# tspooner/rl_markets

Hardware: AMD Instinct MI355X
Metric: env-steps/sec (whole node) at 65 536 parallel books (higher is better)
Workload: dtype f64

## Files before the change

rl_markets_amd/csrc/lob_env.h:

```cpp
#ifndef LOB_ENV_H
#define LOB_ENV_H

#include <hip/hip_runtime.h>

#include "lob_internal.h"
#include "lob_state.h"

LOB_HD int drec_pad4(int n) { return (n + 3) & ~3; }
LOB_HD int drec_words(int D, int T) { return 4 + 4 * drec_pad4(D) + drec_pad4(2 * T); }
LOB_HD int drec_ask_px(int, int) { return 4; }
LOB_HD int drec_ask_vol(int D, int) { return 4 + drec_pad4(D); }
LOB_HD int drec_bid_px(int D, int) { return 4 + 2 * drec_pad4(D); }
LOB_HD int drec_bid_vol(int D, int) { return 4 + 3 * drec_pad4(D); }
LOB_HD int drec_trades(int D, int) { return 4 + 4 * drec_pad4(D); }
LOB_HD void drec_from_abi(const uint32_t* src, int D, int T, uint32_t* dst) {
    const int Wd = drec_words(D, T);
    for (int i = 0; i < Wd; i++) dst[i] = 0;
    dst[0] = src[LOB_REC_TIME];
    dst[1] = src[LOB_REC_FLAGS];
    for (int l = 0; l < D; l++) {
        dst[drec_ask_px(D, T) + l] = src[lob_rec_ask_px(D, T) + l];
        dst[drec_ask_vol(D, T) + l] = src[lob_rec_ask_vol(D, T) + l];
        dst[drec_bid_px(D, T) + l] = src[lob_rec_bid_px(D, T) + l];
        dst[drec_bid_vol(D, T) + l] = src[lob_rec_bid_vol(D, T) + l];
// ... 70 lines not shown
    __device__ const uint32_t* row(int i) const { return rows + (size_t)i * (size_t)P.Wd; }
    __device__ const Track& track(int k) const { return S.track[(size_t)b * (size_t)S.track_len + (size_t)(k & S.track_mask)]; }
    __device__ const TrackHead& track_head(int k) const { return *reinterpret_cast<const TrackHead*>(&track(k)); }
    __device__ const TrackHead64& track_head64(int k) const { return *reinterpret_cast<const TrackHead64*>(&track(k)); }
    __device__ Track& track_w(int k) const { return S.track[(size_t)b * (size_t)S.track_len + (size_t)(k & S.track_mask)]; }
};

__device__ inline f64 key4(f64 p) { return rint(p * 10000.0); }

__device__ inline i64 cvt_long_x86(f64 d) {
    if (!(d >= -9223372036854775808.0 && d < 9223372036854775808.0)) return (i64)0x8000000000000000ull;
    return (i64)d;
}

struct OrderR {
    i64 size, qh, qt, ex;
};
__device__ inline i64 ord_remaining(const OrderR& o) { i64 r = o.size - o.ex; return r > 0 ? r : 0; }
__device__ inline bool ord_executed(const OrderR& o) { return o.ex >= o.size; }
__device__ inline i64 ord_transaction(OrderR& o, i64 volume) {
    i64 remaining_volume = volume - o.qh;
    if (remaining_volume > 0) {
        o.qh = 0;
        if (ord_remaining(o) <= remaining_volume) {
            o.ex = o.size;
            remaining_volume -= o.size;
        } else {
            o.ex += remaining_volume;
            remaining_volume = 0;
        }
    } else {
        o.qh -= volume;
    }
    return remaining_volume > 0 ? remaining_volume : 0;
}
__device__ inline void ord_cancellation(OrderR& o, i64 volume) {
    if (o.qt == 0) {
        o.qh -= volume;
    } else {
        f64 total = (f64)(o.qh + o.qt);
        i64 nh = cvt_long_x86((f64)o.qh - ceil((f64)(volume * o.qh) / total));
        i64 nt = cvt_long_x86((f64)o.qt - floor((f64)(volume * o.qt) / total));
        o.qh = nh;
        o.qt = nt;
    }
    if (o.qh < 0) {
        o.qt = (i64)((u64)o.qt + (u64)o.qh);
        o.qh = 0;
    }
    if (o.qt < 0) o.qt = 0;
}

__device__ inline void rm_push(const RMPtrs& r, int B, int b, f64 val) {
    i32 cnt = r.cnt[b], head = r.head[b];
    f64 sum = r.sum[b], mean = r.mean[b], s = r.s[b];
    sum += val;
    if (cnt < r.w) {
        head = (cnt == 0) ? 0 : (head + 1 == r.w ? 0 : head + 1);
        cnt++;
        r.ring[(size_t)head * B + b] = val;
        f64 n = (f64)cnt;
        f64 old_mean = mean;
        mean += (val - mean) / n;
        s += (val - mean) * (val - old_mean);
    } else {
        i32 oldest = head + 1 == r.w ? 0 : head + 1;
        f64 old = r.ring[(size_t)oldest * B + b];
        r.ring[(size_t)oldest * B + b] = val;
        head = oldest;
        f64 n = (f64)(cnt + 1);
        f64 old_mean = mean;
        mean += (val - mean) / n;
        s += (val - mean) * (val - old_mean);
        sum -= old;
        f64 n2 = (f64)cnt;
        f64 old_mean2 = mean;
        mean -= (old - mean) / n2;
        s -= (old - mean) * (old - old_mean2);
    }
    r.cnt[b] = cnt;
    r.head[b] = head;
    r.sum[b] = sum;
    r.mean[b] = mean;
    r.s[b] = s;
}
__device__ inline f64 rm_front(const RMPtrs& r, int B, int b) { return r.ring[(size_t)r.head[b] * B + b]; }
__device__ inline f64 rm_back(const RMPtrs& r, int B, int b) {
    i32 idx = r.head[b] - r.cnt[b] + 1;
    if (idx < 0) idx += r.w;
    return r.ring[(size_t)idx * B + b];
}
__device__ inline bool rm_full(const RMPtrs& r, int b) { return r.cnt[b] == r.w; }
__device__ inline f64 rm_std(const RMPtrs& r, int b) {
    f64 v = r.s[b] / (f64)(r.cnt[b] - 1);
    return v > 0 ? sqrt(v) : 0.0;
}
__device__ inline void acc_push(const AccPtrs& r, int B, int b, f64 val) {
    i32 cnt = r.cnt[b], head = r.head[b];
    f64 sum = r.sum[b];
    sum += val;
    if (cnt < r.w) {
        head = (cnt == 0) ? 0 : (head + 1 == r.w ? 0 : head + 1);
        cnt++;
        r.ring[(size_t)head * B + b] = val;
    } else {
        i32 oldest = head + 1 == r.w ? 0 : head + 1;
        f64 old = r.ring[(size_t)oldest * B + b];
        r.ring[(size_t)oldest * B + b] = val;
        head = oldest;
        sum -= old;
    }
    r.cnt[b] = cnt;
    r.head[b] = head;
    r.sum[b] = sum;
}

struct RMReg {
    i32 cnt, head, slot;
    f64 sum, mean, s, old;
};
__device__ inline void rm_load(const RMPtrs& r, int b, RMReg& g) {
    g.cnt = r.cnt[b]; g.head = r.head[b]; g.sum = r.sum[b]; g.mean = r.mean[b]; g.s = r.s[b];
}
__device__ inline void rm_prep(const RMPtrs& r, int B, int b, RMReg& g) {
    if (g.cnt < r.w) {
        g.slot = (g.cnt == 0) ? 0 : (g.head + 1 == r.w ? 0 : g.head + 1);
        g.old = 0.0;
    } else {
        g.slot = g.head + 1 == r.w ? 0 : g.head + 1;
        g.old = r.ring[(size_t)g.slot * B + b];
    }
}
__device__ inline void rm_apply(const RMPtrs& r, int B, int b, RMReg& g, f64 val) {
    g.sum += val;
    r.ring[(size_t)g.slot * B + b] = val;
    if (g.cnt < r.w) {
        g.cnt++;
        f64 n = (f64)g.cnt;
        f64 old_mean = g.mean;
        g.mean += (val - g.mean) / n;
        g.s += (val - g.mean) * (val - old_mean);
    } else {
        f64 n = (f64)(g.cnt + 1);
        f64 old_mean = g.mean;
        g.mean += (val - g.mean) / n;
        g.s += (val - g.mean) * (val - old_mean);
        g.sum -= g.old;
        f64 n2 = (f64)g.cnt;
        f64 old_mean2 = g.mean;
        g.mean -= (g.old - g.mean) / n2;
        g.s -= (g.old - g.mean) * (g.old - old_mean2);
    }
    g.head = g.slot;
    r.cnt[b] = g.cnt; r.head[b] = g.head; r.sum[b] = g.sum; r.mean[b] = g.mean; r.s[b] = g.s;
}
__device__ inline void rm_apply_reg(const RMPtrs& r, int B, int b, RMReg& g, f64 val) {
    g.sum += val;
    r.ring[(size_t)g.slot * B + b] = val;
    if (g.cnt < r.w) {
        g.cnt++;
        f64 n = (f64)g.cnt;
        f64 old_mean = g.mean;
        g.mean += (val - g.mean) / n;
        g.s += (val - g.mean) * (val - old_mean);
    } else {
        f64 n = (f64)(g.cnt + 1);
        f64 old_mean = g.mean;
        g.mean += (val - g.mean) / n;
        g.s += (val - g.mean) * (val - old_mean);
        g.sum -= g.old;
        f64 n2 = (f64)g.cnt;
        f64 old_mean2 = g.mean;
        g.mean -= (g.old - g.mean) / n2;
        g.s -= (g.old - g.mean) * (g.old - old_mean2);
    }
    g.head = g.slot;
}
__device__ inline void rm_store(const RMPtrs& r, int b, const RMReg& g) {
    r.cnt[b] = g.cnt; r.head[b] = g.head; r.sum[b] = g.sum; r.mean[b] = g.mean; r.s[b] = g.s;
}
struct AccReg {
    i32 cnt, head, slot;
    f64 sum, old;
};
__device__ inline void acc_load(const AccPtrs& r, int b, AccReg& g) { g.cnt = r.cnt[b]; g.head = r.head[b]; g.sum = r.sum[b]; }
__device__ inline void acc_prep(const AccPtrs& r, int B, int b, AccReg& g) {
    if (g.cnt < r.w) { g.slot = (g.cnt == 0) ? 0 : (g.head + 1 == r.w ? 0 : g.head + 1); g.old = 0.0; }
    else { g.slot = g.head + 1 == r.w ? 0 : g.head + 1; g.old = r.ring[(size_t)g.slot * B + b]; }
}
__device__ inline void acc_apply(const AccPtrs& r, int B, int b, AccReg& g, f64 val) {
    g.sum += val;
    r.ring[(size_t)g.slot * B + b] = val;
    if (g.cnt < r.w) g.cnt++;
    else g.sum -= g.old;
    g.head = g.slot;
    r.cnt[b] = g.cnt; r.head[b] = g.head; r.sum[b] = g.sum;
}

__device__ inline void acc_apply_reg(const AccPtrs& r, int B, int b, AccReg& g, f64 val) {
    g.sum += val;
    r.ring[(size_t)g.slot * B + b] = val;
    if (g.cnt < r.w) g.cnt++;
    else g.sum -= g.old;
    g.head = g.slot;
}
__device__ inline void acc_store(const AccPtrs& r, int b, const AccReg& g) { r.cnt[b] = g.cnt; r.head[b] = g.head; r.sum[b] = g.sum; }

__device__ inline f64 rec_price(const EnvCtx& c, int rec, int side, int l) {
    if (rec < 0) return 0.0;
    const uint32_t* r = c.row(rec);
    return (f64)__uint_as_float(r[(side == 0 ? drec_ask_px(c.P.D, c.P.T) : drec_bid_px(c.P.D, c.P.T)) + l]);
}
__device__ inline int book_level_of(const uint32_t* px, int D, f64 k) {
    uint32_t w[LOB_MAX_DEPTH];
    drec_levels(px, D, w);
    f32 p[LOB_MAX_DEPTH];
#pragma unroll
    for (int l = 0; l < LOB_MAX_DEPTH; l++) p[l] = l < D ? __uint_as_float(w[l]) : 0.0f;
    int hit = -1;
#pragma unroll
    for (int l = 0; l < LOB_MAX_DEPTH; l++)
        if (p[l] != 0.0f && key4((f64)p[l]) == k) hit = l;
    return hit;
}
__device__ inline i64 book_volume(const EnvCtx& c, int rec, int side, f64 price) {
    if (rec < 0) return 0;
    const uint32_t* r = c.row(rec);
    const uint32_t* px = r + (side == 0 ? drec_ask_px(c.P.D, c.P.T) : drec_bid_px(c.P.D, c.P.T));
    const uint32_t* vol = r + (side == 0 ? drec_ask_vol(c.P.D, c.P.T) : drec_bid_vol(c.P.D, c.P.T));
    const int hit = book_level_of(px, c.P.D, key4(price));
    return hit >= 0 ? (i64)(i32)vol[hit] : 0;
}
__device__ inline void book_volume2(const EnvCtx& c, int rec_a, int rec_b, int side, f64 price, i64& va, i64& vb) {
    const int opx = side == 0 ? drec_ask_px(c.P.D, c.P.T) : drec_bid_px(c.P.D, c.P.T);
    const int ovol = side == 0 ? drec_ask_vol(c.P.D, c.P.T) : drec_bid_vol(c.P.D, c.P.T);
    const uint32_t* ra = c.row(rec_a < 0 ? 0 : rec_a);
    const uint32_t* rb = c.row(rec_b < 0 ? 0 : rec_b);
    const int D = c.P.D;
    const f64 k = key4(price);
    uint32_t wa[LOB_MAX_DEPTH], wb[LOB_MAX_DEPTH];
    drec_levels(ra + opx, D, wa);
    drec_levels(rb + opx, D, wb);
    f32 pa[LOB_MAX_DEPTH], pb[LOB_MAX_DEPTH];
#pragma unroll
    for (int l = 0; l < LOB_MAX_DEPTH; l++) {
        pa[l] = l < D ? __uint_as_float(wa[l]) : 0.0f;
        pb[l] = l < D ? __uint_as_float(wb[l]) : 0.0f;
    }
    int ha = -1, hb = -1;
#pragma unroll
    for (int l = 0; l < LOB_MAX_DEPTH; l++) {
        if (pa[l] != 0.0f && key4((f64)pa[l]) == k) ha = l;
        if (pb[l] != 0.0f && key4((f64)pb[l]) == k) hb = l;
    }
    va = (rec_a >= 0 && ha >= 0) ? (i64)(i32)ra[ovol + ha] : 0;
    vb = (rec_b >= 0 && hb >= 0) ? (i64)(i32)rb[ovol + hb] : 0;
}

__device__ inline void order_volumes(const EnvCtx& c, const EnvR& e, int last_rec, int row_rec, i64& a_lv, i64& a_v,
                                     i64& b_lv, i64& b_v) {
    a_lv = a_v = b_lv = b_v = 0;
    const int D = c.P.D;
    const int apx = drec_ask_px(D, c.P.T), avol = drec_ask_vol(D, c.P.T);
    const int bpx = drec_bid_px(D, c.P.T), bvol = drec_bid_vol(D, c.P.T);
    const uint32_t* rl = c.row(last_rec < 0 ? 0 : last_rec);
    const uint32_t* rr = c.row(row_rec < 0 ? 0 : row_rec);
    const bool a_on = e.a_on != 0, b_on = e.b_on != 0;
    uint32_t wal[LOB_MAX_DEPTH], war[LOB_MAX_DEPTH], wbl[LOB_MAX_DEPTH], wbr[LOB_MAX_DEPTH];
    drec_levels(rl + apx, D, wal); drec_levels(rr + apx, D, war);
    drec_levels(rl + bpx, D, wbl); drec_levels(rr + bpx, D, wbr);
    f32 pal[LOB_MAX_DEPTH], par[LOB_MAX_DEPTH], pbl[LOB_MAX_DEPTH], pbr[LOB_MAX_DEPTH];
#pragma unroll
    for (int l = 0; l < LOB_MAX_DEPTH; l++) {
        pal[l] = (a_on && l < D) ? __uint_as_float(wal[l]) : 0.0f;
        par[l] = (a_on && l < D) ? __uint_as_float(war[l]) : 0.0f;
        pbl[l] = (b_on && l < D) ? __uint_as_float(wbl[l]) : 0.0f;
        pbr[l] = (b_on && l < D) ? __uint_as_float(wbr[l]) : 0.0f;
    }
    const f64 ka = key4(e.a_opx), kb = key4(e.b_opx);
    int hal = -1, har = -1, hbl = -1, hbr = -1;
#pragma unroll
    for (int l = 0; l < LOB_MAX_DEPTH; l++) {
        if (pal[l] != 0.0f && key4((f64)pal[l]) == ka) hal = l;
        if (par[l] != 0.0f && key4((f64)par[l]) == ka) har = l;
        if (pbl[l] != 0.0f && key4((f64)pbl[l]) == kb) hbl = l;
        if (pbr[l] != 0.0f && key4((f64)pbr[l]) == kb) hbr = l;
    }
    if (last_rec >= 0 && hal >= 0) a_lv = (i64)(i32)rl[avol + hal];
    if (row_rec >= 0 && har >= 0) a_v = (i64)(i32)rr[avol + har];
    if (last_rec >= 0 && hbl >= 0) b_lv = (i64)(i32)rl[bvol + hbl];
    if (row_rec >= 0 && hbr >= 0) b_v = (i64)(i32)rr[bvol + hbr];
}

struct RowFull {
    uint32_t apx[LOB_MAX_DEPTH], avol[LOB_MAX_DEPTH], bpx[LOB_MAX_DEPTH], bvol[LOB_MAX_DEPTH];
};
__device__ inline void row_full_load(const EnvCtx& c, int rec, RowFull& R) {
    const int D = c.P.D;
    const uint32_t* r = c.row(rec < 0 ? 0 : rec);
    drec_levels(r + drec_ask_px(D, c.P.T), D, R.apx);
    drec_levels(r + drec_ask_vol(D, c.P.T), D, R.avol);
    drec_levels(r + drec_bid_px(D, c.P.T), D, R.bpx);
    drec_levels(r + drec_bid_vol(D, c.P.T), D, R.bvol);
    const uint32_t keep = rec < 0 ? 0u : ~0u;
#pragma unroll
    for (int l = 0; l < LOB_MAX_DEPTH; l++) { R.apx[l] &= keep; R.avol[l] &= keep; R.bpx[l] &= keep; R.bvol[l] &= keep; }
}
__device__ inline void row_volumes(const EnvCtx& c, const EnvR& e, const RowFull& L, i64& a_v, i64& b_v) {
    const int D = c.P.D;
    const bool a_on = e.a_on != 0, b_on = e.b_on != 0;
    const f64 ka = key4(e.a_opx), kb = key4(e.b_opx);
    int ha = -1, hb = -1;
#pragma unroll
    for (int l = 0; l < LOB_MAX_DEPTH; l++) {
        const f32 pa = (a_on && l < D) ? __uint_as_float(L.apx[l]) : 0.0f;
        const f32 pb = (b_on && l < D) ? __uint_as_float(L.bpx[l]) : 0.0f;
        if (pa != 0.0f && key4((f64)pa) == ka) ha = l;
        if (pb != 0.0f && key4((f64)pb) == kb) hb = l;
    }
    uint32_t va = 0, vb = 0;
#pragma unroll
    for (int l = 0; l < LOB_MAX_DEPTH; l++) {
        if (l == ha) va = L.avol[l];
        if (l == hb) vb = L.bvol[l];
    }
    a_v = ha >= 0 ? (i64)(i32)va : 0;
    b_v = hb >= 0 ? (i64)(i32)vb : 0;
}

__device__ inline i64 full_volume(const EnvCtx& c, const RowFull& R, int side, f64 price) {
    const int D = c.P.D;
    const f64 k = key4(price);
    bool hit = false;
    uint32_t v = 0;
#pragma unroll
    for (int l = 0; l < LOB_MAX_DEPTH; l++) {
        const f32 p = l < D ? __uint_as_float(side == 0 ? R.apx[l] : R.bpx[l]) : 0.0f;
        if (p != 0.0f && key4((f64)p) == k) { hit = true; v = side == 0 ? R.avol[l] : R.bvol[l]; }
    }
    return hit ? (i64)(i32)v : 0;
}

__device__ inline void row_resolve(const EnvCtx&, const RowFull&) {}
__device__ inline f64 row_best_px(const RowFull& R, int side) { return (f64)__uint_as_float(side == 0 ? R.apx[0] : R.bpx[0]); }

#if defined(__HIP__)
struct RowLev {
    mutable uint4 q;
    mutable uint32_t apx, avol, bpx, bvol;
    uint32_t* stage;
    int li;
    mutable bool pending;
    bool none;
    __device__ __forceinline__ void resolve(const EnvCtx& c) const {
        if (!pending) return;
        const int D = c.P.D, D4 = drec_pad4(D);
        if (li < (c.P.Wd >> 2)) reinterpret_cast<uint4*>(stage)[li] = q;
        __builtin_amdgcn_fence(__ATOMIC_ACQ_REL, "workgroup", "local");
        __builtin_amdgcn_wave_barrier();
        const bool in = li < D && !none;
        const int l = li < D ? li : 0;
        const uint32_t a = stage[4 + l], av = stage[4 + D4 + l], b = stage[4 + 2 * D4 + l], bv = stage[4 + 3 * D4 + l];
        apx = in ? a : 0u; avol = in ? av : 0u; bpx = in ? b : 0u; bvol = in ? bv : 0u;
        __builtin_amdgcn_fence(__ATOMIC_ACQ_REL, "workgroup", "local");
        __builtin_amdgcn_wave_barrier();
        pending = false;
    }
};
__device__ __forceinline__ uint32_t grp_ballot(bool p) { return (uint32_t)(__ballot(p) >> (threadIdx.x & 48)) & 0xffffu; }
__device__ inline void row_full_load(const EnvCtx& c, int rec, RowLev& R) {
    const uint4* r = reinterpret_cast<const uint4*>(c.row(rec < 0 ? 0 : rec));
    const int nq = c.P.Wd >> 2;
    R.q = r[R.li < nq ? R.li : nq - 1];
    R.none = rec < 0;
    R.pending = true;
}
__device__ inline void row_resolve(const EnvCtx& c, const RowLev& R) { R.resolve(c); }
__device__ inline f64 row_best_px(const RowLev& R, int side) {
    return (f64)__uint_as_float(__shfl(side == 0 ? R.apx : R.bpx, 0, 16));
}
__device__ inline i64 rowlev_volume(const EnvCtx& c, const RowLev& R, int side, f64 k) {
    R.resolve(c);
    const f32 p = __uint_as_float(side == 0 ? R.apx : R.bpx);
    const uint32_t m = grp_ballot(p != 0.0f && key4((f64)p) == k);
    const uint32_t v = __shfl(side == 0 ? R.avol : R.bvol, m ? 31 - __clz(m) : 0, 16);
    return m ? (i64)(i32)v : 0;
}
__device__ inline i64 full_volume(const EnvCtx& c, const RowLev& R, int side, f64 price) { return rowlev_volume(c, R, side, key4(price)); }
__device__ inline void row_volumes_k(const EnvCtx& c, bool a_on, bool b_on, f64 ka, f64 kb, const RowLev& L, i64& a_v, i64& b_v) {
    const i64 va = rowlev_volume(c, L, 0, ka), vb = rowlev_volume(c, L, 1, kb);
    a_v = a_on ? va : 0;
    b_v = b_on ? vb : 0;
}
#endif

__device__ inline void check_orders(const DevParams& P, EnvR& e) {
    if (e.position >= P.pos_ub) e.b_on = 0;
    else if (e.position <= P.pos_lb) e.a_on = 0;
}

template <class ROW>
__device__ inline void place_one(const EnvCtx& c, EnvR& e, int side, f64 price, i32 price_ticks, const ROW& cur) {
    if (!(price > 0.0)) c.err(LOB_ERR_BAD_ORDER_PRICE);
    i64 qh = full_volume(c, cur, side, price);
    if (side == 0) {
        e.a_on = 1; e.a_opx = price; e.a_osz = c.P.order_size; e.a_oqh = qh; e.a_oqt = 0; e.a_oex = 0; e.a_oiq = qh; e.a_otk = price_ticks;
    } else {
        e.b_on = 1; e.b_opx = price; e.b_osz = c.P.order_size; e.b_oqh = qh; e.b_oqt = 0; e.b_oex = 0; e.b_oiq = qh; e.b_otk = price_ticks;
    }
}

template <class ROW>
__device__ inline void place_orders(const EnvCtx& c, EnvR& e, int al, int bl, const ROW& cur) {
    const DevParams& P = c.P;
    e.ask_level = al;
    e.bid_level = bl;
    int ta, tb;
    int band = 0, band_t = 0;
    if (P.quote_mode == LOB_QUOTE_BOOK) {
        row_resolve(c, cur);
        const f64 ap0 = row_best_px(cur, 0), bp0 = row_best_px(cur, 1);
        if (ap0 == 0.0 || bp0 == 0.0) c.err(LOB_ERR_UNDEF_PRICE);
        ta = lobh::to_ticks_hint((*c.tk), ap0, band) + al;
        tb = lobh::to_ticks_hint((*c.tk), bp0, band) - bl;
    } else {
        const Track& t = c.pre_prev ? *c.pre_prev : c.track(e.k - 1);
        f64 tp = t.tp_val;
        f64 half = t.spread_mean / 2.0;
        f64 half_spd = 0.0 > half ? 0.0 : half;
        ta = lobh::to_ticks_hint((*c.tk), tp + (f64)al * half_spd, band);
        tb = lobh::to_ticks_hint((*c.tk), tp - (f64)bl * half_spd, band);
    }
    e.ask_quote = lobh::to_price_hint((*c.tk), ta, band_t);
    e.bid_quote = lobh::to_price_hint((*c.tk), tb, band_t);
    place_one(c, e, 0, e.ask_quote, lobh::to_ticks_hint((*c.tk), e.ask_quote, band), cur);
    place_one(c, e, 1, e.bid_quote, lobh::to_ticks_hint((*c.tk), e.bid_quote, band), cur);
}
__device__ inline void place_orders(const EnvCtx& c, EnvR& e, int al, int bl) {
    RowFull cur;
    row_full_load(c, e.rec_cur, cur);
    place_orders(c, e, al, bl, cur);
}

__device__ inline void market_order(const EnvCtx& c, EnvR& e, i64 size, i64& out_vol, f64& out_proxy, f64& out_value, const RowFull& cur) {
    out_vol = 0; out_proxy = 0.0; out_value = 0.0;
    if (e.rec_cur < 0) c.err(LOB_ERR_UNDEF_PRICE);
    const f64 mip = e.mid;
    if (size == 0) return;
    const int side = size > 0 ? 0 : 1;
    i64 abs_size = size < 0 ? -size : size;
    i64 tv;
    if (e.done == 2) {
        tv = side == 0 ? c.S.prep[c.b].a_tv : c.S.prep[c.b].b_tv;
    } else {
        tv = c.pre_prev ? (side == 0 ? c.pre_prev->a_tv : c.pre_prev->b_tv) : (side == 0 ? c.track(e.k - 1).a_tv : c.track(e.k - 1).b_tv);
    }
    if (abs_size > tv) return;
    i64 executed = 0;
    f64 proxy = 0.0, value = 0.0;
    bool filled = false;
#pragma unroll
    for (int l = 0; l < LOB_MAX_DEPTH; l++) {
        const f32 pf = __uint_as_float(side == 0 ? cur.apx[l] : cur.bpx[l]);
        if (l >= c.P.D || filled || pf == 0.0f) continue;
        f64 p = (f64)pf;
        i64 lvol = (i64)(i32)(side == 0 ? cur.avol[l] : cur.bvol[l]);
        i64 left = abs_size - executed;
        i64 l_ex = lvol < left ? lvol : left;
        executed += l_ex;
        proxy -= (f64)l_ex * fabs(p - mip);
        if (side == 0) value -= (f64)l_ex * p;
        else value += (f64)l_ex * p;
        if (executed >= abs_size) {
            if (side == 0) e.a_ntr++; else e.b_ntr++;
            filled = true;
        }
    }
    out_vol = side == 0 ? executed : -executed;
    out_proxy = proxy;
    out_value = value;
}

#if defined(__HIP__)
__device__ inline void market_order(const EnvCtx& c, EnvR& e, i64 size, i64& out_vol, f64& out_proxy, f64& out_value, const RowLev& cur) {
    out_vol = 0; out_proxy = 0.0; out_value = 0.0;
    if (e.rec_cur < 0) c.err(LOB_ERR_UNDEF_PRICE);
    const f64 mip = e.mid;
    if (size == 0) return;
    const int side = size > 0 ? 0 : 1;
    const i64 abs_size = size < 0 ? -size : size;
    i64 tv;
    if (e.done == 2) tv = side == 0 ? c.S.prep[c.b].a_tv : c.S.prep[c.b].b_tv;
    else tv = c.pre_prev ? (side == 0 ? c.pre_prev->a_tv : c.pre_prev->b_tv) : (side == 0 ? c.track(e.k - 1).a_tv : c.track(e.k - 1).b_tv);
    if (abs_size > tv) return;
    cur.resolve(c);
    const f32 pf = __uint_as_float(side == 0 ? cur.apx : cur.bpx);
    const bool level = cur.li < c.P.D && pf != 0.0f;
    const i64 lvol = level ? (i64)(i32)(side == 0 ? cur.avol : cur.bvol) : 0;
    i64 incl = lvol;
#pragma unroll
    for (int d = 1; d < 16; d <<= 1) {
        const i64 up = __shfl_up(incl, d, 16);
        if (cur.li >= d) incl += up;
    }
    const i64 before = incl - lvol;
    const bool takes = level && before < abs_size;
    const i64 left = abs_size - before;
    const i64 l_ex = takes ? (lvol < left ? lvol : left) : 0;
    const uint32_t fills = grp_ballot(takes && before + l_ex >= abs_size);
    const i64 total = __shfl(incl, 15, 16);
    const i64 executed = total < abs_size ? total : abs_size;
    const f64 p = (f64)pf;
    const f64 t_proxy = takes ? (f64)l_ex * fabs(p - mip) : 0.0;
    const f64 t_value = takes ? (f64)l_ex * p : 0.0;
    f64 proxy = 0.0, value = 0.0;
    for (int l = 0; l < c.P.D; l++) {
        const f64 tp = __shfl(t_proxy, l, 16), tvl = __shfl(t_value, l, 16);
        proxy -= tp;
        if (side == 0) value -= tvl;
        else value += tvl;
    }
    if (fills) { if (side == 0) e.a_ntr++; else e.b_ntr++; }
    out_vol = side == 0 ? executed : -executed;
    out_proxy = proxy;
    out_value = value;
}
#endif

template <class ROW>
__device__ inline void clear_inventory(const EnvCtx& c, EnvR& e, const ROW& cur) {
    i64 v; f64 proxy, value;
    market_order(c, e, -e.position, v, proxy, value, cur);
    e.position += v;
    e.pnl_step += proxy;
    e.lo_vol_step += (i32)(v < 0 ? -v : v);
    e.ep_pnl += value;
    if (v > 0) e.market_buys++;
    else if (v < 0) e.market_sells++;
}
__device__ inline void clear_inventory(const EnvCtx& c, EnvR& e) {
    RowFull cur;
    row_full_load(c, e.rec_cur, cur);
    clear_inventory(c, e, cur);
}

template <class ROW>
__device__ inline void do_action(const EnvCtx& c, EnvR& e, int action, const ROW& cur) {
    int al, bl;
    switch (action) {
        case 0: al = 1; bl = 1; break;
        case 1: clear_inventory(c, e, cur); al = e.ask_level; bl = e.bid_level; break;
        case 2: al = 2; bl = 2; break;
        case 3: al = 3; bl = 3; break;
        case 4: al = 0; bl = 2; break;
        case 5: al = 2; bl = 0; break;
        case 6: al = 1; bl = 4; break;
        case 7: al = 4; bl = 1; break;
        case 8: al = 5; bl = 5; break;
        default: return;
    }
    place_orders(c, e, al, bl, cur);
}

__device__ inline bool is_open(const DevParams& P, i32 t) {
    return ((i64)t > P.open_ms + 30 * 60000LL) && ((i64)t < P.close_ms - 30 * 60000LL);
}

__device__ inline f32 expf_glibc(f32 x) {
    static const u64 T[32] = {
        0x3ff0000000000000ull, 0x3fefd9b0d3158574ull, 0x3fefb5586cf9890full, 0x3fef9301d0125b51ull, 0x3fef72b83c7d517bull,
        0x3fef54873168b9aaull, 0x3fef387a6e756238ull, 0x3fef1e9df51fdee1ull, 0x3fef06fe0a31b715ull, 0x3feef1a7373aa9cbull,
        0x3feedea64c123422ull, 0x3feece086061892dull, 0x3feebfdad5362a27ull, 0x3feeb42b569d4f82ull, 0x3feeab07dd485429ull,
        0x3feea47eb03a5585ull, 0x3feea09e667f3bcdull, 0x3fee9f75e8ec5f74ull, 0x3feea11473eb0187ull, 0x3feea589994cce13ull,
        0x3feeace5422aa0dbull, 0x3feeb737b0cdc5e5ull, 0x3feec49182a3f090ull, 0x3feed503b23e255dull, 0x3feee89f995ad3adull,
        0x3feeff76f2fb5e47ull, 0x3fef199bdd85529cull, 0x3fef3720dcef9069ull, 0x3fef5818dcfba487ull, 0x3fef7c97337b9b5full,
        0x3fefa4afa2a490daull, 0x3fefd0765b6e4540ull};
    const f64 N = 32.0;
    const f64 InvLn2N = 0x1.71547652b82fep+0 * N, SHIFT = 0x1.8p+52;
    const f64 C0 = 0x1.c6af84b912394p-5 / N / N / N, C1 = 0x1.ebfce50fac4f3p-3 / N / N, C2 = 0x1.62e42ff0c52d6p-1 / N;
    const uint32_t ux = __float_as_uint(x), ax = ux & 0x7fffffffu;
    if (ax >= 0x42b00000u) {
        if (ux == 0xff800000u) return 0.0f;
        if (ax >= 0x7f800000u) return x + x;
        if (x > 0x1.62e42ep6f) return __uint_as_float(0x7f800000u);
        if (x < -0x1.9fe368p6f) return 0.0f;
    }
    const f64 xd = (f64)x;
    f64 kd = fma(InvLn2N, xd, SHIFT);
    const u64 ki = (u64)__double_as_longlong(kd);
    kd -= SHIFT;
    const f64 r = fma(InvLn2N, xd, -kd);
    const f64 s = __longlong_as_double((long long)(T[ki % 32] + (ki << 47)));
    const f64 z = fma(C0, r, C1);
    const f64 r2 = r * r;
    f64 y = fma(C2, r, 1.0);
    y = fma(z, r2, y);
    y = y * s;
    return (f32)y;
}

__device__ inline f64 get_reward(const EnvCtx& c, const EnvR& e, const f64* spread_mean = nullptr) {
    const DevParams& P = c.P;
    f64 r = 0.0;
    i64 ap = e.position < 0 ? -e.position : e.position;
    i32 abs_pos = (i32)ap;
    switch (P.reward_measure) {
// ... 1255 lines not shown
```

rl_markets_amd/csrc/lob_envstep.h:

```cpp
#ifndef LOB_ENVSTEP_H
#define LOB_ENVSTEP_H

#include "lob_fast.h"

__device__ inline Track track_load(const Track* p) {
    const uint4* q = reinterpret_cast<const uint4*>(p);
    uint4 w[8];
#pragma unroll
    for (int i = 0; i < 8; i++) w[i] = q[i];
    Track t;
    uint4* d = reinterpret_cast<uint4*>(&t);
#pragma unroll
    for (int i = 0; i < 8; i++) d[i] = w[i];
    return t;
}

template <int LANES> struct EnvStepOcc { static constexpr int waves = LANES == 64 ? 1 : 2; };
template <bool INLINE_GENERAL, bool DQ = false, int LANES = 64>
__global__ void __launch_bounds__(64, EnvStepOcc<LANES>::waves) env_step_kernel(const DevParams* __restrict__ Pp, const DevState* __restrict__ Sp, int step_id, int par, EnvFuse F,
                                                                                  const uint32_t* __restrict__ rnd_g) {
    static_assert(LANES == 64 || !INLINE_GENERAL, "the half-full variant leaves the books without a list to the work list");
    const DevParams& P = *Pp;
    const DevState& S = *Sp;
    __shared__ TickLds tick_lds;
    __shared__ EnvSlot lds_env[LANES == 64 ? 64 : LANES + 1];
    __shared__ LearnLds1 lds_learn;
#ifdef LOB_PROF
    const long long t_entry = clock64();
#else
    const long long t_entry = 0;
#endif
    const int t = blockIdx.x * LANES + (int)threadIdx.x;
    const bool valid = (int)threadIdx.x < LANES && t < S.B;
    const int b = valid ? t : S.B - 1;
    const int B = S.B;

    f64 tk_lb = 0.0, tk_tick = 0.0, tk_pp = 0.0;
    i64 tk_cum = 0;
    i32 tk_pt = 0;
    if (threadIdx.x < LOB_MAX_BANDS) {
        const int i = threadIdx.x;
        tk_lb = P.band_lb[i]; tk_tick = P.band_tick[i]; tk_cum = P.band_cum[i]; tk_pp = P.band_pp[i]; tk_pt = P.band_pt[i];
    }
    EnvCtx c(P, S, b, &tick_lds);
    LHdr* hp = S.hdr + b;
    const LHdr h0 = *hp;
    const int k0 = S.k[b], rc0 = S.rec_cur[b];
    const int mslot = S.mk_slot[b];
    const bool dirty = S.hl_dirty[0] == F.sid_prev;
    constexpr int HLQ = LOB_HL_ROW / 2;
    ulonglong2 hl[HLQ];
    const ulonglong2* hl_p = reinterpret_cast<const ulonglong2*>(S.hl_rec + (size_t)b * LOB_HL_REC);
#pragma unroll
    for (int i = 0; i < HLQ; i++) hl[i] = i < 8 ? hl_p[i] : make_ulonglong2(0ull, 0ull);
    EnvR er;
    env_load(S, b, er);
    RMReg wu, wd;
    rm_load(S.pnl_ups, b, wu);
    rm_load(S.pnl_downs, b, wd);
    const int m_n_track = S.meta[b].n_track, m_complete = S.meta[b].complete;

    if (threadIdx.x < LOB_MAX_BANDS) {
        const int i = threadIdx.x;
        tick_lds.lb[i] = tk_lb; tick_lds.tick[i] = tk_tick; tick_lds.cum[i] = tk_cum; tick_lds.pp[i] = tk_pp; tick_lds.pt[i] = tk_pt;
    }
    if (threadIdx.x == 0) tick_lds.n = P.n_bands;
    EnvR& e = lds_env[LANES == 64 || threadIdx.x < LANES ? (threadIdx.x & (LANES - 1)) : LANES].e;
    if (LANES == 64 || threadIdx.x < LANES) e = er;
    __syncthreads();
#ifdef LOB_PROF
    const long long t_r1 = clock64();
#endif

    const int cur_slot = h0.slot_cur ^ 1;
    const bool alive = valid && !h0.done;
    const bool open = is_open(P, h0.time_ms);
    const int n_list = hl[0].x == LOB_HL_NONE ? -1 : (int)hl[0].x;
    bool ok = alive && open && !dirty && !((h0.zero_mask >> (cur_slot ^ 1)) & 1) && mslot >= 0 && n_list >= 0;
    if (ok && n_list > 15) {
#pragma unroll
        for (int i = 8; i < HLQ; i++) hl[i] = hl_p[i];
    }

    const int ms = mslot >= 0 ? mslot : 0;
    const MemoRec rec = *reinterpret_cast<const MemoRec*>(S.mk_rec + ((size_t)S.mk_slots + ms) * LOB_MK_REC);
    const int tiles_ok = S.mk_tiles_ok[ms];
    const uint32_t mk_bits = S.mk_marked[ms];
#define LOB_HL_ENT(i) (((1 + (i)) & 1) ? hl[(1 + (i)) >> 1].y : hl[(1 + (i)) >> 1].x)
    f64 wv[LOB_HL_CAP];
#pragma unroll
    for (int i = 0; i < LOB_HL_CAP; i++) {
        wv[i] = 0.0;
        if (ok && i < n_list) wv[i] = S.theta[(uint32_t)LOB_HL_ENT(i)];
    }
    f64 wvb[DQ ? LOB_HL_CAP : 1];
    f64 s0b[DQ ? LOB_N_ACTIONS : 1];
    if (DQ) {
        const f64* recb = S.mk_rec_b + ((size_t)S.mk_slots + ms) * LOB_MK_REC;
#pragma unroll
        for (int a = 0; a < LOB_N_ACTIONS; a++) s0b[DQ ? a : 0] = recb[a];
#pragma unroll
        for (int i = 0; i < LOB_HL_CAP; i++) {
            wvb[DQ ? i : 0] = 0.0;
            if (ok && i < n_list) wvb[DQ ? i : 0] = S.theta_b[(uint32_t)LOB_HL_ENT(i)];
        }
    }
    const int kk = k0 > 0 ? k0 : 1;
    Track tprev;
    {
        const uint4* q = reinterpret_cast<const uint4*>(&c.track(kk - 1));
        const uint4 w4 = q[4], w5 = q[5];
        uint4* d = reinterpret_cast<uint4*>(&tprev);
#pragma unroll
        for (int i = 0; i < 8; i++) d[i] = make_uint4(0, 0, 0, 0);
        d[4] = w4; d[5] = w5;
    }
    Track tcur = track_load(&c.track(k0));
    RowFull cur, first;
    row_full_load(c, rc0, cur);
    {
        const int last_row = S.events_of(b) - 1;
        row_full_load(c, rc0 + 1 < last_row ? rc0 + 1 : last_row, first);
    }
    rm_prep(S.pnl_ups, B, b, wu);
    rm_prep(S.pnl_downs, B, b, wd);
#ifdef LOB_PROF
    __builtin_amdgcn_s_waitcnt(0);
    const long long t_r2 = clock64();
#endif

    int action = 0;
    bool go = false;
    if (valid) {
        if (h0.done) {
            hp->stepped = 0;
        } else if (!open) {
            hp->slot_cur = cur_slot; hp->done = 1; hp->stepped = 0; S.done[b] = 1;
        } else {
            ok = ok && rec.ver == F.ver;
            if (!ok) {
                if (!INLINE_GENERAL) {
                    const int pos = atomicAdd(&S.slow_n[F.lpar * 2 + 0], 1);
                    S.slow_list[pos] = b;
                }
            } else {
                f64 q[LOB_N_ACTIONS];
#pragma unroll
                for (int a = 0; a < LOB_N_ACTIONS; a++) q[a] = rec.s0[a];
                const f64 w1 = P.w1, w2 = P.w2;
#pragma unroll
                for (int i = 0; i < LOB_HL_CAP; i++) {
                    const u64 ent = LOB_HL_ENT(i);
                    const f64 v = wv[i];
                    if (i < n_list && v != 0.0) {
                        const int a_ = (int)(ent >> 32) & 15;
                        const f64 x_ = ((ent >> 36) & 1ull ? w2 : w1) * v;
#pragma unroll
                        for (int a = 0; a < LOB_N_ACTIONS; a++) q[a] = a_ == a ? q[a] + x_ : q[a];
                    }
                }
                constexpr int NT = LOB_HL_MAX - LOB_HL_CAP;
                u64 te[NT];
                if (n_list > LOB_HL_CAP) {
                    const u64* tp = S.hl_rec + (size_t)b * LOB_HL_REC + 1 + LOB_HL_CAP;
#pragma unroll
                    for (int j = 0; j < NT; j++) te[j] = LOB_HL_CAP + j < n_list ? tp[j] : 0ull;
                    f64 tv[NT];
#pragma unroll
                    for (int j = 0; j < NT; j++) tv[j] = LOB_HL_CAP + j < n_list ? S.theta[(uint32_t)te[j]] : 0.0;
#pragma unroll
                    for (int j = 0; j < NT; j++) {
                        if (LOB_HL_CAP + j < n_list && tv[j] != 0.0) {
                            const int a_ = (int)(te[j] >> 32) & 15;
                            const f64 x_ = ((te[j] >> 36) & 1ull ? w2 : w1) * tv[j];
#pragma unroll
                            for (int a = 0; a < LOB_N_ACTIONS; a++) q[a] = a_ == a ? q[a] + x_ : q[a];
                        }
                    }
                }
#pragma unroll
                for (int a = 0; a < LOB_N_ACTIONS; a++) S.qs_last[(size_t)b * LOB_N_ACTIONS + a] = q[a];
                if (DQ) {
                    f64 qb[LOB_N_ACTIONS];
#pragma unroll
                    for (int a = 0; a < LOB_N_ACTIONS; a++) qb[a] = s0b[DQ ? a : 0];
#pragma unroll
                    for (int i = 0; i < LOB_HL_CAP; i++) {
                        const u64 ent = LOB_HL_ENT(i);
                        const f64 v = wvb[DQ ? i : 0];
                        if (i < n_list && v != 0.0) {
                            const int a_ = (int)(ent >> 32) & 15;
                            const f64 x_ = ((ent >> 36) & 1ull ? w2 : w1) * v;
#pragma unroll
                            for (int a = 0; a < LOB_N_ACTIONS; a++) qb[a] = a_ == a ? qb[a] + x_ : qb[a];
                        }
                    }
                    if (n_list > LOB_HL_CAP) {
                        f64 tv[NT];
#pragma unroll
                        for (int j = 0; j < NT; j++) tv[j] = LOB_HL_CAP + j < n_list ? S.theta_b[(uint32_t)te[j]] : 0.0;
#pragma unroll
                        for (int j = 0; j < NT; j++) {
                            if (LOB_HL_CAP + j < n_list && tv[j] != 0.0) {
                                const int a_ = (int)(te[j] >> 32) & 15;
                                const f64 x_ = ((te[j] >> 36) & 1ull ? w2 : w1) * tv[j];
#pragma unroll
                                for (int a = 0; a < LOB_N_ACTIONS; a++) qb[a] = a_ == a ? qb[a] + x_ : qb[a];
                            }
                        }
                    }
#pragma unroll
                    for (int a = 0; a < LOB_N_ACTIONS; a++) {
                        S.qs_last_b[(size_t)b * LOB_N_ACTIONS + a] = qb[a];
                        q[a] = (q[a] + qb[a]) / 2.0;
                    }
                }
                Rng g{P.seed, P.book_id_offset + (u64)b, h0.rng_ctr};
                action = policy_sample(P, q, false, g);
                hp->slot_cur = cur_slot;
                hp->action = action;
                hp->stepped = 1;
                hp->rng_ctr = g.ctr;
                const uint32_t marked = tiles_ok ? mk_bits : 0x1ffu;
                if (!((marked >> action) & 1u)) {
                    const int pos = atomicAdd(&S.mk_markcount[0], 1);
                    if (pos < S.mk_slots) S.mk_marklist[pos] = mslot * 16 + action;
                    else mark_generation(P, S, mslot, action);
                    atomicOr(&S.mk_marked[mslot], 1u << action);
                }
                const u64 act = __ballot(1);
                if ((int)(threadIdx.x & 63) == __builtin_ctzll(act)) cnt_add(S, 5, (unsigned long long)__builtin_popcountll(act));
                go = true;
            }
        }
    }
#undef LOB_HL_ENT
    if (INLINE_GENERAL) {
        u64 todo = __ballot(valid && alive && open && !ok);
        if (todo) {
            if (threadIdx.x == 0) cnt_add(S, 2, (u64)__builtin_popcountll(todo));
            const uint4* src = reinterpret_cast<const uint4*>(rnd_g);
            uint4* dst = reinterpret_cast<uint4*>(lds_learn.rnd);
            for (int i = threadIdx.x; i < 512; i += 64) dst[i] = src[i];
            if (threadIdx.x < 27) lds_learn.act_terms[threadIdx.x] = rnd_g[2048 + threadIdx.x];
            wave_lds_fence();
            while (todo) {
                const int src_lane = __builtin_ctzll(todo);
                todo &= todo - 1;
                const int b_src = __builtin_amdgcn_readlane(b, src_lane);
                int act = -1;
                act_book<DQ ? LOB_ALGO_DOUBLE_Q : LOB_ALGO_SARSA, LearnLds1>(P, S, lds_learn, 0, (int)threadIdx.x, b_src, 0, par, &act);
                if ((int)threadIdx.x == src_lane && act >= 0) { action = act; go = true; }
            }
        }
    }

    i64 d_steps = 0, d_events = 0;
    if (go) {
        c.pre_prev = &tprev;
        c.pre_n_track = m_n_track;
        c.pre_complete = m_complete;
        c.prof_start(S.prof, threadIdx.x & 63, t_entry);
#ifdef LOB_PROF
        c.acc_[0] += t_r1 - t_entry;
        c.acc_[11] += t_r2 - t_r1;
        c.pt_ = t_r2;
#endif
        c.mark(30);
        const i64 ev0 = e.events;
        StepAgg g;
        step_prologue(c, e, action, g, cur);
        const int st = event_loop_fast(c, e, g, tcur, first);
        bool claim = false;
        u64 claim_k = 0;
        int claim_stamp = 0, claim_slot_prev = -1, claim_q0 = 0, claim_q1 = 0, claim_q2 = 0;
        d_events = e.events - ev0;
        if (st != 2) {
            step_epilogue_pre(c, e, g, wu, wd);
            const int cs = cur_slot;
            f32* v = S.vars + ((size_t)b * 3 + cs) * 16;
            f32* vf = S.vars + ((size_t)b * 3 + 2) * 16;
            int qg[3] = {0, 0, 0};
            for (int i = 0; i < P.V; i++) {
                v[i] = (f32)get_variable(c, e, P.vars[i], tcur);
                vf[i] = v[i];
                if (i < 3) qg[i] = tile_quant(v[i]);
            }
            if (P.memo) {
                const uint32_t s0 = (uint32_t)mk_hash3(qg[0], qg[1], qg[2]) & (uint32_t)(S.mk_slots - 1);
                claim_k = S.mk_hash[s0];
                claim_stamp = S.mk_stamp[s0];
                claim_slot_prev = mslot;
                claim_q0 = qg[0]; claim_q1 = qg[1]; claim_q2 = qg[2];
                claim = true;
            }
            hp->zero_mask = h0.zero_mask & ~(1 << cs);
            S.verdict[(size_t)b * LOB_VD_STRIDE + 67] = 0;
            hp->reward = get_reward(c, e, &tcur.spread_mean);
            hp->stepped = 1;
            d_steps = 1;
        } else {
            hp->stepped = 0;
        }
        c.mark(28);
        hp->done = e.done;
        hp->time_ms = e.time_ms;
        env_store(S, b, e);
        if (claim) {
            S.mk_slot_last[b] = claim_slot_prev;
            S.mk_slot[b] = mk_claim(S, claim_q0, claim_q1, claim_q2, step_id, par, claim_k, claim_stamp);
        }
        c.mark(29);
        c.flush();
    }
    for (int off = 32; off > 0; off >>= 1) {
        d_steps += __shfl_down(d_steps, off);
        d_events += __shfl_down(d_events, off);
    }
    if ((threadIdx.x & 63) == 0 && (d_steps | d_events)) {
        cnt_add(S, 0, (u64)d_steps);
        cnt_add(S, 1, (u64)d_events);
        cnt_add(S, 3, (u64)d_steps);
    }
}


#define LOB_ENV16_BOOKS 4
template <bool INLINE_GENERAL>
__global__ void __launch_bounds__(64) env_step16_kernel(const DevParams* __restrict__ Pp, const DevState* __restrict__ Sp, int step_id, int par, EnvFuse F,
                                                        const uint32_t* __restrict__ rnd_g) {
    const DevParams& P = *Pp;
    const DevState& S = *Sp;
    __shared__ TickLds tick_lds;
    __shared__ __align__(16) uint32_t lds_row[LOB_ENV16_BOOKS][64];
    __shared__ LearnLds1 lds_learn;
    const int grp = (int)threadIdx.x >> 4, li = (int)threadIdx.x & 15;
    const bool lead = li == 0;
    const int t = blockIdx.x * LOB_ENV16_BOOKS + grp;
    const bool valid = t < S.B;
    const int b = valid ? t : S.B - 1;
    const int B = S.B;

    if (threadIdx.x < LOB_MAX_BANDS) {
        const int i = threadIdx.x;
        tick_lds.lb[i] = P.band_lb[i]; tick_lds.tick[i] = P.band_tick[i]; tick_lds.cum[i] = P.band_cum[i]; tick_lds.pp[i] = P.band_pp[i]; tick_lds.pt[i] = P.band_pt[i];
    }
    if (threadIdx.x == 0) tick_lds.n = P.n_bands;
    EnvCtx c(P, S, b, &tick_lds);
    LHdr* hp = S.hdr + b;
    const LHdr h0 = *hp;
    const int k0 = S.k[b], rc0 = S.rec_cur[b];
    const int mslot = S.mk_slot[b];
    const bool dirty = S.hl_dirty[0] == F.sid_prev;
    const u64* hl_p = S.hl_rec + (size_t)b * LOB_HL_REC;
    const u64 hl_n = hl_p[0];
    u64 ent[3];
#pragma unroll
    for (int j = 0; j < 3; j++) ent[j] = 16 * j + li < LOB_HL_MAX ? hl_p[1 + 16 * j + li] : 0ull;
    EnvR er;
    env_load(S, b, er);
    RMReg wu, wd;
    rm_load(S.pnl_ups, b, wu);
    rm_load(S.pnl_downs, b, wd);
    const int m_n_track = S.meta[b].n_track, m_complete = S.meta[b].complete;
    EnvR e = er;
    __syncthreads();

    const int cur_slot = h0.slot_cur ^ 1;
    const bool alive = valid && !h0.done;
    const bool open = is_open(P, h0.time_ms);
    const int n_list = hl_n == LOB_HL_NONE ? -1 : (int)hl_n;
    bool ok = alive && open && !dirty && !((h0.zero_mask >> (cur_slot ^ 1)) & 1) && mslot >= 0 && n_list >= 0;

    const int ms = mslot >= 0 ? mslot : 0;
    const MemoRec rec = *reinterpret_cast<const MemoRec*>(S.mk_rec + ((size_t)S.mk_slots + ms) * LOB_MK_REC);
    const int tiles_ok = S.mk_tiles_ok[ms];
    const uint32_t mk_bits = S.mk_marked[ms];
    f64 wv[3];
#pragma unroll
    for (int j = 0; j < 3; j++) wv[j] = (ok && 16 * j + li < n_list) ? S.theta[(uint32_t)ent[j]] : 0.0;
    const int kk = k0 > 0 ? k0 : 1;
    Track tprev;
    {
        const uint4* q = reinterpret_cast<const uint4*>(&c.track(kk - 1));
        const uint4 w4 = q[4], w5 = q[5];
        uint4* d = reinterpret_cast<uint4*>(&tprev);
#pragma unroll
        for (int i = 0; i < 8; i++) d[i] = make_uint4(0, 0, 0, 0);
        d[4] = w4; d[5] = w5;
    }
    Track tcur = track_load(&c.track(k0));
    RowLev cur, first;
    cur.stage = first.stage = lds_row[grp];
    cur.li = first.li = li;
    cur.pending = first.pending = false;
    row_full_load(c, rc0, cur);
    {
        const int last_row = S.events_of(b) - 1;
        row_full_load(c, rc0 + 1 < last_row ? rc0 + 1 : last_row, first);
    }
    rm_prep(S.pnl_ups, B, b, wu);
    rm_prep(S.pnl_downs, B, b, wd);

    int action = 0;
    bool go = false;
    if (valid) {
        if (h0.done) {
            if (lead) hp->stepped = 0;
        } else if (!open) {
            if (lead) { hp->slot_cur = cur_slot; hp->done = 1; hp->stepped = 0; S.done[b] = 1; }
        } else {
            ok = ok && rec.ver == F.ver;
            if (!ok) {
                if (!INLINE_GENERAL && lead) {
                    const int pos = atomicAdd(&S.slow_n[F.lpar * 2 + 0], 1);
                    S.slow_list[pos] = b;
                }
            } else {
                f64 q[LOB_N_ACTIONS];
#pragma unroll
                for (int a = 0; a < LOB_N_ACTIONS; a++) q[a] = rec.s0[a];
                const f64 w1 = P.w1, w2 = P.w2;
                for (int j = 0; j < n_list; j++) {
                    const int jj = j >> 4;
                    const u64 en = __shfl(jj == 0 ? ent[0] : jj == 1 ? ent[1] : ent[2], j & 15, 16);
// ... 118 lines not shown
```

Before: 286.2 million.

## Coalesce per-book record loads via wave-cooperative fetch and LDS transpose

In the non-DQ path, each lane's header, hot-list, memo record, track and two order-book rows are no longer loaded as strided per-thread vectors. The wave now fetches them cooperatively with shuffled base addresses, so adjacent lanes read contiguous 16-byte chunks of the same record. The data is then transposed through LDS, reusing the learn scratch buffer, back into per-lane registers. This is meant to cut uncoalesced global traffic, at the cost of extra shuffles, LDS round-trips, fences and register pressure.

Result: slower. 280.4 million, median of 6 (-2.0%).

```diff
diff --git a/rl_markets_amd/csrc/lob_env.h b/rl_markets_amd/csrc/lob_env.h
--- a/rl_markets_amd/csrc/lob_env.h
+++ b/rl_markets_amd/csrc/lob_env.h
@@ -396,6 +396,18 @@
     drec_levels(r + drec_ask_vol(D, c.P.T), D, R.avol);
     drec_levels(r + drec_bid_px(D, c.P.T), D, R.bpx);
     drec_levels(r + drec_bid_vol(D, c.P.T), D, R.bvol);
+    const uint32_t keep = rec < 0 ? 0u : ~0u;
+#pragma unroll
+    for (int l = 0; l < LOB_MAX_DEPTH; l++) { R.apx[l] &= keep; R.avol[l] &= keep; R.bpx[l] &= keep; R.bvol[l] &= keep; }
+}
+#define LOB_ROW_SPAN_QUADS (4 * LOB_LEVEL_QUADS)
+__device__ inline const uint32_t* row_span(const EnvCtx& c, int rec) { return c.row(rec < 0 ? 0 : rec) + drec_ask_px(c.P.D, c.P.T); }
+__device__ inline void row_full_unpack(const EnvCtx& c, int rec, const uint4* span, RowFull& R) {
+    const int D = c.P.D, a4 = drec_pad4(D) / 4;
+    drec_unpack(span, D, R.apx);
+    drec_unpack(span + a4, D, R.avol);
+    drec_unpack(span + 2 * a4, D, R.bpx);
+    drec_unpack(span + 3 * a4, D, R.bvol);
     const uint32_t keep = rec < 0 ? 0u : ~0u;
 #pragma unroll
     for (int l = 0; l < LOB_MAX_DEPTH; l++) { R.apx[l] &= keep; R.avol[l] &= keep; R.bpx[l] &= keep; R.bvol[l] &= keep; }
diff --git a/rl_markets_amd/csrc/lob_envstep.h b/rl_markets_amd/csrc/lob_envstep.h
--- a/rl_markets_amd/csrc/lob_envstep.h
+++ b/rl_markets_amd/csrc/lob_envstep.h
@@ -13,6 +13,39 @@
 #pragma unroll
     for (int i = 0; i < 8; i++) d[i] = w[i];
     return t;
+}
+
+typedef uint32_t q32x4 __attribute__((ext_vector_type(4)));
+typedef __attribute__((address_space(1))) const q32x4 gq32x4;
+template <int NQ>
+__device__ inline void wave_quads_fetch(const void* rec, q32x4 (&v)[NQ]) {
+    const u64 a = (u64)rec;
+    const int lane = (int)threadIdx.x & 63;
+#pragma unroll
+    for (int j = 0; j < NQ; j++) {
+        const int i = 64 * j + lane, o = i / NQ;
+        v[j] = *((const gq32x4*)__shfl(a, o) + (i - o * NQ));
+    }
+}
+template <int NQ> struct WaveStage { static constexpr int stride = NQ | 1, quads = 64 * stride; };
+template <int NQ>
+__device__ inline const uint4* wave_quads_stage(const q32x4 (&v)[NQ], q32x4* stage) {
+    const int lane = (int)threadIdx.x & 63;
+    wave_lds_fence();
+#pragma unroll
+    for (int j = 0; j < NQ; j++) {
+        const int i = 64 * j + lane, o = i / NQ;
+        stage[o * WaveStage<NQ>::stride + (i - o * NQ)] = v[j];
+    }
+    wave_lds_fence();
+    return reinterpret_cast<const uint4*>(stage + lane * WaveStage<NQ>::stride);
+}
+template <class T>
+__device__ inline void quads_to(const uint4* src, T& dst) {
+    static_assert(sizeof(T) % 16 == 0, "whole quads");
+    uint4* d = reinterpret_cast<uint4*>(&dst);
+#pragma unroll
+    for (int i = 0; i < (int)(sizeof(T) / 16); i++) d[i] = src[i];
 }
 
 template <int LANES> struct EnvStepOcc { static constexpr int waves = LANES == 64 ? 1 : 2; };
@@ -24,7 +57,7 @@
     const DevState& S = *Sp;
     __shared__ TickLds tick_lds;
     __shared__ EnvSlot lds_env[LANES == 64 ? 64 : LANES + 1];
-    __shared__ LearnLds1 lds_learn;
+    __shared__ __align__(16) LearnLds1 lds_learn;
 #ifdef LOB_PROF
     const long long t_entry = clock64();
 #else
@@ -44,21 +77,37 @@
     }
     EnvCtx c(P, S, b, &tick_lds);
     LHdr* hp = S.hdr + b;
-    const LHdr h0 = *hp;
+    constexpr bool WAVE = !DQ;
+    constexpr int HLQ = LOB_HL_ROW / 2;
+    const ulonglong2* hl_p = reinterpret_cast<const ulonglong2*>(S.hl_rec + (size_t)b * LOB_HL_REC);
+    q32x4 v_hdr[sizeof(LHdr) / 16], v_hl[8];
+    if constexpr (WAVE) {
+        wave_quads_fetch(hp, v_hdr);
+        wave_quads_fetch(hl_p, v_hl);
+    }
     const int k0 = S.k[b], rc0 = S.rec_cur[b];
     const int mslot = S.mk_slot[b];
     const bool dirty = S.hl_dirty[0] == F.sid_prev;
-    constexpr int HLQ = LOB_HL_ROW / 2;
-    ulonglong2 hl[HLQ];
-    const ulonglong2* hl_p = reinterpret_cast<const ulonglong2*>(S.hl_rec + (size_t)b * LOB_HL_REC);
-#pragma unroll
-    for (int i = 0; i < HLQ; i++) hl[i] = i < 8 ? hl_p[i] : make_ulonglong2(0ull, 0ull);
     EnvR er;
     env_load(S, b, er);
     RMReg wu, wd;
     rm_load(S.pnl_ups, b, wu);
     rm_load(S.pnl_downs, b, wd);
     const int m_n_track = S.meta[b].n_track, m_complete = S.meta[b].complete;
+    q32x4* stage = reinterpret_cast<q32x4*>(&lds_learn);
+    static_assert(WaveStage<LOB_ROW_SPAN_QUADS>::quads * 16 <= sizeof(LearnLds1), "the largest record's staging fits LearnLds1");
+    LHdr h0;
+    ulonglong2 hl[HLQ];
+    if constexpr (WAVE) {
+        quads_to(wave_quads_stage(v_hdr, stage), h0);
+        const ulonglong2* own = reinterpret_cast<const ulonglong2*>(wave_quads_stage(v_hl, stage));
+#pragma unroll
+        for (int i = 0; i < HLQ; i++) hl[i] = i < 8 ? own[i] : make_ulonglong2(0ull, 0ull);
+    } else {
+        h0 = *hp;
+#pragma unroll
+        for (int i = 0; i < HLQ; i++) hl[i] = i < 8 ? hl_p[i] : make_ulonglong2(0ull, 0ull);
+    }
 
     if (threadIdx.x < LOB_MAX_BANDS) {
         const int i = threadIdx.x;
@@ -83,7 +132,12 @@
     }
 
     const int ms = mslot >= 0 ? mslot : 0;
-    const MemoRec rec = *reinterpret_cast<const MemoRec*>(S.mk_rec + ((size_t)S.mk_slots + ms) * LOB_MK_REC);
+    const int kk = k0 > 0 ? k0 : 1;
+    const int last_row = S.events_of(b) - 1, rc1 = rc0 + 1 < last_row ? rc0 + 1 : last_row;
+    constexpr int MQ = sizeof(MemoRec) / 16;
+    q32x4 v_rec[MQ], v_prev[2], v_cur[sizeof(Track) / 16], v_row0[LOB_ROW_SPAN_QUADS], v_row1[LOB_ROW_SPAN_QUADS];
+    const f64* rec_p = S.mk_rec + ((size_t)S.mk_slots + ms) * LOB_MK_REC;
+    if constexpr (WAVE) wave_quads_fetch(rec_p, v_rec);
     const int tiles_ok = S.mk_tiles_ok[ms];
     const uint32_t mk_bits = S.mk_marked[ms];
 #define LOB_HL_ENT(i) (((1 + (i)) & 1) ? hl[(1 + (i)) >> 1].y : hl[(1 + (i)) >> 1].x)
@@ -94,33 +148,49 @@
         if (ok && i < n_list) wv[i] = S.theta[(uint32_t)LOB_HL_ENT(i)];
     }
     f64 wvb[DQ ? LOB_HL_CAP : 1];
+    if (DQ) {
+#pragma unroll
+        for (int i = 0; i < LOB_HL_CAP; i++) {
+            wvb[DQ ? i : 0] = 0.0;
+            if (ok && i < n_list) wvb[DQ ? i : 0] = S.theta_b[(uint32_t)LOB_HL_ENT(i)];
+        }
+    }
     f64 s0b[DQ ? LOB_N_ACTIONS : 1];
     if (DQ) {
         const f64* recb = S.mk_rec_b + ((size_t)S.mk_slots + ms) * LOB_MK_REC;
 #pragma unroll
         for (int a = 0; a < LOB_N_ACTIONS; a++) s0b[DQ ? a : 0] = recb[a];
-#pragma unroll
-        for (int i = 0; i < LOB_HL_CAP; i++) {
-            wvb[DQ ? i : 0] = 0.0;
-            if (ok && i < n_list) wvb[DQ ? i : 0] = S.theta_b[(uint32_t)LOB_HL_ENT(i)];
-        }
-    }
-    const int kk = k0 > 0 ? k0 : 1;
-    Track tprev;
+    }
+    const uint4* prev_p = reinterpret_cast<const uint4*>(&c.track(kk - 1)) + 4;
+    MemoRec rec;
+    Track tprev, tcur;
+    RowFull cur, first;
     {
-        const uint4* q = reinterpret_cast<const uint4*>(&c.track(kk - 1));
-        const uint4 w4 = q[4], w5 = q[5];
         uint4* d = reinterpret_cast<uint4*>(&tprev);
 #pragma unroll
         for (int i = 0; i < 8; i++) d[i] = make_uint4(0, 0, 0, 0);
-        d[4] = w4; d[5] = w5;
-    }
-    Track tcur = track_load(&c.track(k0));
-    RowFull cur, first;
-    row_full_load(c, rc0, cur);
-    {
-        const int last_row = S.events_of(b) - 1;
-        row_full_load(c, rc0 + 1 < last_row ? rc0 + 1 : last_row, first);
+    }
+    if constexpr (WAVE) {
+        wave_quads_fetch(prev_p, v_prev);
+        wave_quads_fetch(&c.track(k0), v_cur);
+        wave_quads_fetch(row_span(c, rc0), v_row0);
+        wave_quads_fetch(row_span(c, rc1), v_row1);
+        quads_to(wave_quads_stage(v_rec, stage), rec);
+        const uint4* own = wave_quads_stage(v_prev, stage);
+        reinterpret_cast<uint4*>(&tprev)[4] = own[0];
+        reinterpret_cast<uint4*>(&tprev)[5] = own[1];
+        quads_to(wave_quads_stage(v_cur, stage), tcur);
+        row_full_unpack(c, rc0, wave_quads_stage(v_row0, stage), cur);
+        row_full_unpack(c, rc1, wave_quads_stage(v_row1, stage), first);
+        wave_lds_fence();
+    } else {
+        rec = *reinterpret_cast<const MemoRec*>(rec_p);
+        const uint4 w4 = prev_p[0], w5 = prev_p[1];
+        reinterpret_cast<uint4*>(&tprev)[4] = w4;
+        reinterpret_cast<uint4*>(&tprev)[5] = w5;
+        tcur = track_load(&c.track(k0));
+        row_full_load(c, rc0, cur);
+        row_full_load(c, rc1, first);
     }
     rm_prep(S.pnl_ups, B, b, wu);
     rm_prep(S.pnl_downs, B, b, wd);
```
